# pingcap/tidb

Hardware: NVIDIA H100
Metric: hash-join probe rows/sec (higher is better)
Workload: dtype int64

## Files before the change

### tidb_b200/csrc/join.cu

```cuda
#include <memory>
#include <deque>
#include <algorithm>
#include <cmath>
#include <condition_variable>
#include "join_kernels.cuh"
#include "partition_kernels.cuh"
#include "chunk_io.cuh"

namespace tg {

static const int64_t kGeneralBatchRows = 16ll << 20;
static const int64_t kDirectPushRows = 128ll << 10;
static const int64_t kNextWindowRows = 1ll << 20;

struct Side {
  int ncols = 0;
  std::vector<int> types;
  std::vector<uint32_t> flags;
  std::vector<int> elem;
  std::vector<int> kelem;
  bool has_cells = false;
  std::vector<char> needed;
  int key_col = -1;
  std::vector<int> key_cols;
// ... 358 lines not shown
  return TG_OK;
}

static int kernel_view(JoinImpl* j, const Side& s, DevCols& v, int64_t rows) {
  if (!s.has_cells) return TG_OK;
  TG_TRY(ensure_iota(j, rows));
  for (int c = 0; c < s.ncols; c++)
    if (s.needed[c] && s.elem[c] == kCellBytes) { v.data[c] = j->iota.p; v.elem_len[c] = 8; }
  return TG_OK;
}

struct ProbeTuning { int ctas_per_sm; bool partition; int parts; int part_min_mb; int part_min_rows; int inplace; };
static ProbeTuning probe_tuning() {
  ProbeTuning t;
  t.ctas_per_sm = env_int("TG_PROBE_CTAS_PER_SM", 0);
  t.partition = env_int("TG_PROBE_PARTITION", 1) != 0;
  t.parts = env_int("TG_PROBE_PARTS", 0);
  t.part_min_mb = env_int("TG_PROBE_PART_MIN_MB", 64);
  t.part_min_rows = env_int("TG_PROBE_PART_MIN_ROWS", 1 << 22);
  t.inplace = env_int("TG_PROBE_INPLACE", -1);
  return t;
}

static size_t l2_slice_target(int device) {
  static size_t cache[64];
  if (device >= 0 && device < 64 && cache[device]) return cache[device];
  int l2 = 0;
  if (cudaDeviceGetAttribute(&l2, cudaDevAttrL2CacheSize, device) != cudaSuccess || l2 <= 0) { cudaGetLastError(); l2 = 50 << 20; }
  const size_t t = (size_t)l2 / 4;
  if (device >= 0 && device < 64) cache[device] = t;
  return t;
}
static int probe_slices(size_t table_bytes, int device, int parts_override) {
  if (parts_override > 0) return std::min(parts_override, TG_MAX_PARTS);
  const size_t target = l2_slice_target(device);
  return (int)std::min<size_t>((table_bytes + target - 1) / target, TG_MAX_PARTS);
}
static const double kMaxDenseLoad = 0.5;
static const double kInplaceMinMatch = 0.995;

static const double kPidxLoad = 0.7;
static const double kPidxKeysPerBucket = 4.0;
static const size_t kPidxMaxPilotBytes = 160 << 10;
static int enqueue_scan(JoinImpl* j, int64_t n, int64_t* nblocks_out);
static int build_slice_index(JoinImpl* j, const Slot* slots, unsigned long long nslots) {
  const ProbeTuning& tune = probe_tuning();
  const uint32_t P = (uint32_t)probe_slices((size_t)nslots * sizeof(Slot), j->device, tune.parts);
  if (P < 2) return TG_OK;
  DevBuf cnt;
  TG_TRY(cnt.ensure(j->device, (size_t)(TG_MAX_PARTS + 1) * 8));
  unsigned long long* pcnt = cnt.as<unsigned long long>();
  TG_CUDA(cudaMemsetAsync(pcnt, 0, (size_t)(TG_MAX_PARTS + 1) * 8, j->stream));
  k_pidx_part_count<<<grid_size(j->nsm, (int64_t)nslots, 256, 8), 256, 0, j->stream>>>(slots, nslots, P, pcnt);
  unsigned long long hc[TG_MAX_PARTS];
  TG_CUDA(cudaMemcpyAsync(hc, pcnt, P * 8, cudaMemcpyDeviceToHost, j->stream));
  TG_CUDA(cudaStreamSynchronize(j->stream));
  unsigned long long mx = 0;
  for (uint32_t p = 0; p < P; p++) mx = std::max(mx, hc[p]);
  SliceIndex ix{};
  ix.P = P;
  ix.S = (uint32_t)std::ceil((double)mx / kPidxLoad) + 1;
  ix.B = ((uint32_t)std::ceil((double)mx / kPidxKeysPerBucket) + 16) & ~15u;
  int optin = 0;
  cudaDeviceGetAttribute(&optin, cudaDevAttrMaxSharedMemoryPerBlockOptin, j->device);
  if (ix.B > kPidxMaxPilotBytes || ix.B > (uint32_t)optin) return TG_OK;
  const size_t nb = (size_t)P * ix.B, ns = (size_t)P * ix.S;
  TG_TRY(j->pidx_slots.ensure(j->device, ns * sizeof(Slot)));
  TG_TRY(j->pidx_pilot.ensure(j->device, nb));
  DevBuf owner, list;
  TG_TRY(owner.ensure(j->device, ns * 4));
  TG_TRY(list.ensure(j->device, (size_t)(mx * P + 1) * 4));
  TG_TRY(j->tmp_cnt.ensure(j->device, (nb + 1) * 4));
  Slot* islots = j->pidx_slots.as<Slot>();
  ix.slots = islots;
  ix.pilot = j->pidx_pilot.as<uint8_t>();
  TG_CUDA(cudaMemsetAsync(j->pidx_pilot.p, (int)kPilotNone, nb, j->stream));
  TG_CUDA(cudaMemsetAsync(owner.p, 0xFF, ns * 4, j->stream));
  TG_CUDA(cudaMemsetAsync(j->tmp_cnt.p, 0, (nb + 1) * 4, j->stream));
  k_table_init<<<grid_size(j->nsm, (int64_t)ns, 256, 8), 256, 0, j->stream>>>(islots, ns, ns);
  const unsigned g = (unsigned)grid_size(j->nsm, (int64_t)nslots, 256, 8);
  k_pidx_bucket_count<<<g, 256, 0, j->stream>>>(slots, nslots, ix, j->tmp_cnt.as<uint32_t>());
  int64_t nblocks = 0;
  TG_TRY(enqueue_scan(j, (int64_t)nb, &nblocks));
  const unsigned long long* off = j->tmp_off.as<unsigned long long>();
  k_pidx_lists<<<g, 256, 0, j->stream>>>(slots, nslots, ix, off, j->tmp_cnt.as<uint32_t>(), list.as<uint32_t>());
  const unsigned gb = (unsigned)grid_size(j->nsm, (int64_t)nb, 256, 8);
  for (uint32_t size = kPidxMaxBucket; size >= 1; size--)
    k_pidx_place<<<gb, 256, 0, j->stream>>>(slots, ix, off, list.as<uint32_t>(), size, owner.as<uint32_t>(), j->pidx_pilot.as<uint8_t>());
  unsigned long long* bad = pcnt + TG_MAX_PARTS;
  k_pidx_write<<<g, 256, 0, j->stream>>>(slots, nslots, ix, islots, 0, bad);
  k_pidx_write<<<g, 256, 0, j->stream>>>(slots, nslots, ix, islots, 1, bad);
  j->stats.kernel_launches += 8 + kPidxMaxBucket;
  unsigned long long hbad = 0;
  TG_CUDA(cudaMemcpyAsync(&hbad, bad, 8, cudaMemcpyDeviceToHost, j->stream));
  TG_CUDA(cudaStreamSynchronize(j->stream));
  if (hbad) { j->pidx_slots.release(); j->pidx_pilot.release(); return TG_OK; }
  j->pidx = ix;
  return TG_OK;
}


static int64_t inplace_seg_cap(const JoinImpl* j, int P, int64_t n_main, int64_t C0) {
  if (j->seg_parts != P || j->seg_rows <= 0) return C0;
  const double f = (double)j->seg_fill_max * (double)n_main / (double)j->seg_rows;
  const int64_t C = ((int64_t)(f + 8.0 * std::sqrt(f)) + 4096 + 127) / 128 * 128;
  return std::min(C, C0);
}

static int build_table(JoinImpl* j) {
  const Side& b = j->build;
  int64_t n = j->bcols.rows;
  j->stats.build_rows = n;
  DevCols bview = j->bcols.view(b);
  TG_TRY(kernel_view(j, b, bview, n));
  KeySpec ks = j->build_key;
  if (j->multi_key) {
    TG_TRY(composite_key(j, b, bview, n, j->bkey_syn, j->bkey_syn_nn));
    ks.data = j->bkey_syn.p; ks.nulls = j->bkey_syn_nn.as<uint8_t>();
  } else { ks.data = bview.data[b.key_col]; ks.nulls = bview.nulls[b.key_col]; }
  unsigned long long nslots = (unsigned long long)((double)(n > 0 ? n : 1) / j->load_factor) + 32;
  if (j->default_load_factor) {
    const unsigned long long fit = ((unsigned long long)TG_MAX_PARTS * (33ull << 20)) / sizeof(Slot);
// ... 307 lines not shown
};
template <int NPC, int NKD, int NMD>
struct LaunchSeg {
  static int run(JoinImpl* j, const int64_t* pkey, int64_t n, const FastOut& fo, unsigned long long* cur, const ProbeTuning& t, const SegSpec& seg) {
    static int resident = 0;
    if (!resident) {
      int nb = 0;
      if (cudaOccupancyMaxActiveBlocksPerMultiprocessor(&nb, k_probe_inner_u1_seg_lean<NPC, NKD, NMD>, 256, 0) != cudaSuccess || nb < 1) { cudaGetLastError(); nb = 3; }
      resident = nb;
    }
    int64_t ctas = (n / 128 + 7) / 8;
    int per_sm = t.ctas_per_sm > 0 ? t.ctas_per_sm : resident;
    int grid = (int)std::min<int64_t>(ctas, (int64_t)j->nsm * per_sm);
    k_probe_inner_u1_seg_lean<NPC, NKD, NMD><<<grid, 256, 0, j->stream>>>(pkey, n, j->tv, fo, cur, seg);
    return TG_OK;
  }
};
template <int NPC, int NKD, int NMD>
struct LaunchInplace {
  static int run(JoinImpl* j, int64_t n, const FastOut& fo, unsigned long long* cur, const ProbeTuning& t, const SegSpec& seg, uint32_t* tile_cnt) {
    if constexpr (NKD == 0) {
      return fail(TG_ERR_CUDA, "internal: the in-place segment probe needs an output fed by the join key");
    } else {
      static int resident = 0;
      if (!resident) {
        int nb = 0;
        if (cudaOccupancyMaxActiveBlocksPerMultiprocessor(&nb, k_probe_inner_u1_seg_inplace<NPC, NKD, NMD>, 256, 0) != cudaSuccess || nb < 1) { cudaGetLastError(); nb = 3; }
        resident = nb;
      }
      int64_t ctas = (n / 128 + 7) / 8;
      int per_sm = t.ctas_per_sm > 0 ? t.ctas_per_sm : resident;
      int grid = (int)std::min<int64_t>(ctas, (int64_t)j->nsm * per_sm);
      if (j->pidx.P == (uint32_t)(n / seg.cap)) {
        TG_CUDA(cudaFuncSetAttribute(k_probe_inner_u1_seg_inplace_pidx<NPC, NKD, NMD>, cudaFuncAttributeMaxDynamicSharedMemorySize,
                                     (int)kPidxMaxPilotBytes));
        k_probe_inner_u1_seg_inplace_pidx<NPC, NKD, NMD><<<j->nsm, kPidxThreads, j->pidx.B, j->stream>>>(n, j->tv, j->pidx, fo, cur, seg, tile_cnt);
        j->stats.paths |= TG_JOIN_PATH_PROBE_INDEX;
        return TG_OK;
      }
      k_probe_inner_u1_seg_inplace<NPC, NKD, NMD><<<grid, 256, 0, j->stream>>>(n, j->tv, fo, cur, seg, tile_cnt);
      return TG_OK;
    }
  }
};
static int launch_probe_warp(JoinImpl* j, const int64_t* pkey, int64_t n, const FastOut& fo, unsigned long long* cur, const ProbeTuning& t,
                             const SegSpec& seg = SegSpec{nullptr, 0, 0, 0, nullptr}) {
  j->stats.paths |= TG_JOIN_PATH_PROBE_DIRECT;
  return dispatch_shape<LaunchWarp>(fo, j, pkey, n, fo, cur, t, seg);
}
static int launch_probe_seg(JoinImpl* j, const int64_t* pkey, int64_t n, const FastOut& fo, unsigned long long* cur, const ProbeTuning& t, const SegSpec& seg) {
  j->stats.paths |= TG_JOIN_PATH_PROBE_SEG;
  return dispatch_shape<LaunchSeg>(fo, j, pkey, n, fo, cur, t, seg);
}
static bool aligned16(const void* p) { return (reinterpret_cast<uintptr_t>(p) & 15) == 0; }

static int probe_device(JoinImpl* j, const DevCols& pcells, int64_t n, ResultBatch& rb, bool sync_count, const SegSpec* in_seg = nullptr) {
  const Side& p = j->probe;
  DevCols pview = pcells;
  TG_TRY(kernel_view(j, p, pview, n));
  j->stats.probe_rows += n;
  KeySpec ks = j->probe_key;
  if (j->multi_key) {
    if (in_seg) return fail(TG_ERR_UNSUPPORTED, "segmented device chunks: joins on several key columns take the general path");
    TG_TRY(composite_key(j, p, pview, n, j->pkey_syn, j->pkey_syn_nn));
    ks.data = j->pkey_syn.p; ks.nulls = j->pkey_syn_nn.as<uint8_t>();
  } else { ks.data = pview.data[p.key_col]; ks.nulls = pview.nulls[p.key_col]; }
  TG_TRY(j->out_cursor.ensure(j->device, 64));
  OutCols oc{};
  fill_outspec_probe(j, oc);
// ... 2 lines not shown
  if (in_seg && !fast) return fail(TG_ERR_UNSUPPORTED, "segmented device chunks are only accepted by the fused fast path (unique build keys, <= 1 payload, no filters, an output shape the warp kernels cover)");
  if (fast) {
    const ProbeTuning& tune = probe_tuning();
    const int64_t* pkey = reinterpret_cast<const int64_t*>(ks.data);
    const size_t table_bytes = (size_t)j->tv.nslots * sizeof(Slot);
    bool src16 = aligned16(pkey);
    for (int c = 0; c < fo.n_pcols; c++) src16 = src16 && aligned16(fo.psrc[c]);
    const int64_t PTILE = 1024;
    const int64_t n_main = n / PTILE * PTILE;
    int P = 0;
    int64_t C = 0;
    if (n_main > 0 && tune.partition && src16 && n >= (int64_t)tune.part_min_rows && table_bytes > ((size_t)tune.part_min_mb << 20)) {
      P = probe_slices(table_bytes, j->device, tune.parts);
      C = ((int64_t)((double)n_main / P * 1.05) + 16384 + 127) / 128 * 128;
      if (!(P >= 2 && (int64_t)P * C / 128 < (1ll << 31))) P = 0;
    }
    const bool inplace = P && !in_seg && rb.rows == 0 && fo.n_key_dst >= 1 &&
                         (tune.inplace >= 0 ? tune.inplace != 0 : j->seg_match >= kInplaceMinMatch);
    if (inplace) C = inplace_seg_cap(j, P, n_main, C);
    TG_TRY(ensure_result(j, rb, inplace ? std::max<int64_t>(n, (int64_t)P * C) : rb.rows + n, rb.rows > 0, rb.rows));
    for (int c = 0; c < j->n_out; c++) { oc.data[c] = kernel_out(j, rb, c) + (size_t)rb.rows * 8; oc.valid[c] = nullptr; if (rb.bitmaps[c]->p) rb.bitmaps[c]->release(); }
    build_fast_out(j, oc, pview, fo);
    unsigned long long* cur = j->out_cursor.as<unsigned long long>();
    TG_CUDA(cudaMemsetAsync(cur, 0, 8, j->stream));
    if (n > 0) {
      if (P) {
        const int nc = 1 + fo.n_pcols;
        if (!inplace) {
          for (int c = 0; c < nc; c++) {
            if (!j->part_cols[c]) j->part_cols[c].reset(new DevBuf());
            TG_TRY(j->part_cols[c]->ensure(j->device, (size_t)P * C * 8 + 64));
          }
        }
        TG_TRY(j->part_scratch.ensure(j->device, (size_t)3 * TG_MAX_PARTS * 8 + 64));
        unsigned long long* cursors = j->part_scratch.as<unsigned long long>();
        long long* bases = reinterpret_cast<long long*>(cursors + TG_MAX_PARTS);
        unsigned long long* flag = cursors + 2 * TG_MAX_PARTS;
        PartDst d{};
        d.nparts = P; d.ncols = nc;
        d.src[0] = pkey;
        for (int c = 0; c < fo.n_pcols; c++) d.src[1 + c] = fo.psrc[c];
        for (int c = 0; c < nc; c++)
          for (int q = 0; q < P; q++) d.dst[q][c] = inplace ? (c == 0 ? (void*)fo.key_dst[0] : (void*)fo.pdst[c - 1]) : j->part_cols[c]->p;
        k_segment_bases<<<1, 32, 0, j->stream>>>(cursors, bases, flag, P, C);
        d.dst_base = bases; d.capacity = C; d.overflow = flag;
        if (in_seg) { d.in_cnt = in_seg->cnt; d.in_cap = in_seg->cap; d.in_tiles_per_seg = (uint32_t)(in_seg->cap / PTILE); }
        TG_TRY(launch_partition_scatter<true>(j->device, j->stream, reinterpret_cast<const long long*>(pkey), nullptr, n_main, d, cursors,
                                              &j->stats.kernel_launches, 0, &j->stats.paths));
        const SegSpec seg{cursors, (uint32_t)(C / 128), 0, C, flag};
        if (inplace) {
          const int64_t ntiles = (int64_t)P * C / 128;
          TG_TRY(j->tile_cnt.ensure(j->device, (size_t)ntiles * 4 + 16));
          TG_TRY(j->tmp_cnt.ensure(j->device, (size_t)(2 * ntiles + 1) * 4));
          j->stats.paths |= TG_JOIN_PATH_PROBE_SEG;
          TG_TRY(dispatch_shape<LaunchInplace>(fo, j, (int64_t)P * C, fo, cur, tune, seg, j->tile_cnt.as<uint32_t>()));
          k_inplace_holes<<<grid_size(j->nsm, ntiles, 256, 4), 256, 0, j->stream>>>(j->tile_cnt.as<uint32_t>(), ntiles, cur, flag, j->tmp_cnt.as<uint32_t>());
          int64_t nblocks = 0;
          TG_TRY(enqueue_scan(j, 2 * ntiles, &nblocks));
          k_inplace_fill<<<j->nsm * 8, 256, 0, j->stream>>>(j->tile_cnt.as<uint32_t>(), ntiles, j->tmp_off.as<unsigned long long>(), cur, flag, fo);
          j->stats.kernel_launches += 3;
        } else {
          FastOut pf = fo;
          for (int c = 0; c < fo.n_pcols; c++) pf.psrc[c] = j->part_cols[1 + c]->as<unsigned long long>();
          TG_TRY(launch_probe_seg(j, j->part_cols[0]->as<int64_t>(), (int64_t)P * C, pf, cur, tune, seg));
          j->stats.kernel_launches++;
        }
        if (in_seg) TG_TRY(launch_probe_warp(j, pkey, n_main, fo, cur, tune, SegSpec{in_seg->cnt, in_seg->tiles_per_seg, 1, in_seg->cap, flag, 0}));
        else TG_TRY(launch_probe_warp(j, pkey, n, fo, cur, tune, SegSpec{nullptr, 0, 1, 0, flag, n_main < n ? n_main : 0}));
        j->stats.kernel_launches += 2;
      } else {
        if (in_seg) TG_TRY(launch_probe_warp(j, pkey, n, fo, cur, tune, SegSpec{in_seg->cnt, in_seg->tiles_per_seg, 0, in_seg->cap, nullptr}));
        else TG_TRY(launch_probe_warp(j, pkey, n, fo, cur, tune));
        j->stats.kernel_launches++;
      }
    }
    TG_TRY(gather_cells(j, rb, &pcells, cur));
    if (sync_count) {
      unsigned long long got = 0, part[2 * TG_MAX_PARTS + 1];
      const bool learn = P && !in_seg;
      if (learn) TG_CUDA(cudaMemcpyAsync(part, j->part_scratch.p, sizeof(part), cudaMemcpyDeviceToHost, j->stream));
      TG_CUDA(cudaMemcpyAsync(&got, cur, 8, cudaMemcpyDeviceToHost, j->stream));
      TG_CUDA(cudaStreamSynchronize(j->stream));
      rb.rows += (int64_t)got;
      j->stats.output_rows += (int64_t)got;
      if (P && n > 0) j->seg_match = (double)got / (double)n;
      if (learn) {
        j->seg_parts = part[2 * TG_MAX_PARTS] ? 0 : P;
        j->seg_rows = n_main;
        j->seg_fill_max = (int64_t)*std::max_element(part, part + P);
      }
    }
    return TG_OK;
  }
  if (uq_path_ok(j, pview)) {
    TG_TRY(ensure_result(j, rb, rb.rows + n, rb.rows > 0, rb.rows));
    for (int c = 0; c < j->n_out; c++) { oc.data[c] = kernel_out(j, rb, c) + (size_t)rb.rows * 8; oc.valid[c] = nullptr; if (rb.bitmaps[c]->p) rb.bitmaps[c]->release(); }
    unsigned long long* cur = j->out_cursor.as<unsigned long long>();
    TG_CUDA(cudaMemsetAsync(cur, 0, 8, j->stream));
    if (n > 0) {
      int64_t tiles = (n + 256 * UQ_R - 1) / (256 * UQ_R);
      int grid = (int)std::min<int64_t>(tiles, (int64_t)j->nsm * 8);
      k_probe_inner_uq<<<grid, 256, 0, j->stream>>>(ks, pview, p.filter, n, j->tv, oc, cur);
      j->stats.kernel_launches++;
      j->stats.paths |= TG_JOIN_PATH_PROBE_UQ;
    }
    TG_TRY(gather_cells(j, rb, &pcells, cur));
    unsigned long long got = 0;
    TG_CUDA(cudaMemcpyAsync(&got, cur, 8, cudaMemcpyDeviceToHost, j->stream));
    TG_CUDA(cudaStreamSynchronize(j->stream));
    TG_CUDA(cudaGetLastError());
    rb.rows += (int64_t)got;
    j->stats.output_rows += (int64_t)got;
    return TG_OK;
  }
  std::vector<char> nullable;
  out_nullable(j, pview, nullable);
  if ((int)j->tmp_valid.size() != j->n_out) { j->tmp_valid.clear(); for (int i = 0; i < j->n_out; i++) j->tmp_valid.emplace_back(new DevBuf()); }
  int64_t out_start = rb.rows;
  for (int64_t lo = 0; lo < n || (lo == 0 && n == 0); lo += kGeneralBatchRows) {
    int64_t m = std::min<int64_t>(kGeneralBatchRows, n - lo);
// ... 375 lines not shown
```

### tidb_b200/csrc/join_kernels.cuh

```cuda
#pragma once
#include "common.cuh"
#include "tma.cuh"

namespace tg {

struct __align__(16) Slot { int64_t key; unsigned long long meta; };

static const uint32_t kInvalidSlot = 0xFFFFFFFFu;
static const unsigned long long kCntMask = (1ull << 28) - 1;

enum { TABLE_NONE = 0, TABLE_U1 = 1, TABLE_G = 2 };
enum { KEY_I64 = 0, KEY_F64 = 1, KEY_F32 = 2, KEY_TIME = 3 };
enum { SRC_PROBE_COL = 0, SRC_BUILD_KEY = 1, SRC_BUILD_META = 2, SRC_BUILD_WORD = 3, SRC_FLAG = 4 };

struct KeySpec {
  const void* data;
  const uint8_t* nulls;
  int32_t kind;
  int32_t reject_negative;
};

struct TableView {
  Slot* slots;
  unsigned long long nslots;
// ... 675 lines not shown
#pragma unroll
            for (int d = 1; d < NKD; d++) __stcs(reinterpret_cast<ulonglong2*>(out.key_dst[d] + o), kk);
#pragma unroll
            for (int d = 0; d < NMD; d++) __stcs(reinterpret_cast<ulonglong2*>(out.meta_dst[d] + o), make_ulonglong2(meta[2 * g], meta[2 * g + 1]));
          }
        } else {
          unsigned long long pv[R][NP];
          inplace_load_pv<NPC>(base, out, pv, lane);
          unsigned bal[R];
#pragma unroll
          for (int j = 0; j < R; j++) {
            bal[j] = __ballot_sync(0xffffffffu, (hit >> j) & 1u);
            m += __popc(bal[j]);
          }
          inplace_store<NPC, NKD, NMD>(base, k, meta, pv, bal, out, lane);
        }
      }
    } else if (limit > base) {
      m = inplace_tile_generic<NPC, NKD, NMD>(base, limit, t, out, lane);
    }
    if (lane == 0) tile_cnt[tile] = m;
    kept += m;
  }
  if (lane == 0 && kept) atomicAdd(out_cursor, kept);
}

static constexpr uint32_t kPilotNone = 255;
static constexpr int kPidxMaxBucket = 32;
static constexpr int kPidxThreads = 1024;

struct SliceIndex {
  const Slot* slots;
  const uint8_t* pilot;
  uint32_t P, S, B, pad;
};

__host__ __device__ __forceinline__ uint32_t pidx_slot(uint64_t h, uint32_t q, uint32_t S) {
  return slot32(hash64(h ^ ((uint64_t)(q + 1) * 0xC2B2AE3D27D4EB4Full)), S);
}
__host__ __device__ __forceinline__ uint32_t pidx_bucket(uint64_t h, uint32_t B) { return mulhi32((uint32_t)h, B); }

__global__ void __launch_bounds__(256) k_pidx_part_count(const Slot* __restrict__ slots, unsigned long long nslots, uint32_t P,
                                                         unsigned long long* __restrict__ pcnt) {
  __shared__ unsigned int c[64];
  for (int i = threadIdx.x; i < 64; i += blockDim.x) c[i] = 0;
  __syncthreads();
  for (unsigned long long i = blockIdx.x * (unsigned long long)blockDim.x + threadIdx.x; i < nslots; i += (unsigned long long)gridDim.x * blockDim.x) {
    const int64_t k = slots[i].key;
    if (k != kEmptyKey) atomicAdd(&c[slot32(hash64((uint64_t)k), P)], 1u);
  }
  __syncthreads();
  for (int i = threadIdx.x; i < (int)P; i += blockDim.x) if (c[i]) atomicAdd(&pcnt[i], (unsigned long long)c[i]);
}

__global__ void __launch_bounds__(256) k_pidx_bucket_count(const Slot* __restrict__ slots, unsigned long long nslots, SliceIndex ix,
                                                           uint32_t* __restrict__ bcnt) {
  for (unsigned long long i = blockIdx.x * (unsigned long long)blockDim.x + threadIdx.x; i < nslots; i += (unsigned long long)gridDim.x * blockDim.x) {
    const int64_t k = slots[i].key;
    if (k == kEmptyKey) continue;
    const uint64_t h = hash64((uint64_t)k);
    atomicAdd(&bcnt[(size_t)slot32(h, ix.P) * ix.B + pidx_bucket(h, ix.B)], 1u);
  }
}

__global__ void __launch_bounds__(256) k_pidx_lists(const Slot* __restrict__ slots, unsigned long long nslots, SliceIndex ix,
                                                    const unsigned long long* __restrict__ off, uint32_t* __restrict__ bcnt,
                                                    uint32_t* __restrict__ list) {
// ... 16 lines not shown
    uint64_t h[kPidxMaxBucket];
    for (uint32_t j = 0; j < size; j++) h[j] = hash64((uint64_t)slots[list[o + j]].key);
    uint32_t* const base = owner + (b / ix.B) * ix.S;
    for (uint32_t q = 0; q < kPilotNone; q++) {
      uint32_t won = 0;
      for (; won < size; won++)
        if (atomicCAS(base + pidx_slot(h[won], q, ix.S), 0xFFFFFFFFu, (uint32_t)b) != 0xFFFFFFFFu) break;
      if (won == size) { pilot[b] = (uint8_t)q; break; }
      for (uint32_t j = 0; j < won; j++) atomicExch(base + pidx_slot(h[j], q, ix.S), 0xFFFFFFFFu);
    }
  }
}

__global__ void __launch_bounds__(256) k_pidx_write(const Slot* __restrict__ slots, unsigned long long nslots, SliceIndex ix,
                                                    Slot* __restrict__ islots, int check, unsigned long long* __restrict__ bad) {
  for (unsigned long long i = blockIdx.x * (unsigned long long)blockDim.x + threadIdx.x; i < nslots; i += (unsigned long long)gridDim.x * blockDim.x) {
    const Slot s = slots[i];
    if (s.key == kEmptyKey) continue;
    const uint64_t h = hash64((uint64_t)s.key);
    const uint32_t p = slot32(h, ix.P);
    const uint32_t q = ix.pilot[(size_t)p * ix.B + pidx_bucket(h, ix.B)];
    if (q == kPilotNone) continue;
    Slot* d = islots + (size_t)p * ix.S + pidx_slot(h, q, ix.S);
    if (!check) *d = s;
    else if (d->key != s.key || d->meta != s.meta) atomicAdd(bad, 1ull);
  }
}

template <int NPC, int NKD, int NMD>
__global__ void __launch_bounds__(kPidxThreads, 1)
k_probe_inner_u1_seg_inplace_pidx(int64_t n, TableView t, SliceIndex ix, FastOut out, unsigned long long* __restrict__ out_cursor,
                                  SegSpec seg, uint32_t* __restrict__ tile_cnt) {
  static_assert(NKD >= 1, "the probe key is read from the first key destination");
  constexpr int R = 4, G = 2, NP = NPC > 0 ? NPC : 1;
  extern __shared__ __align__(16) uint8_t spil[];
  if (seg.gate && ((*seg.gate != 0ull) != (seg.gate_want != 0))) return;
  const int lane = threadIdx.x & 31;
  const int64_t warps_total = (int64_t)gridDim.x * (kPidxThreads / 32);
  const int64_t warp_id = (int64_t)blockIdx.x * (kPidxThreads / 32) + (threadIdx.x >> 5);
  const int64_t* __restrict__ pkey = reinterpret_cast<const int64_t*>(out.key_dst[0]);
  const int nseg = (int)(n / 128 / seg.tiles_per_seg);
  unsigned long long kept = 0;
  for (int p = 0; p < nseg; p++) {
    __syncthreads();
    const uint4* src = reinterpret_cast<const uint4*>(ix.pilot + (size_t)p * ix.B);
    for (uint32_t i = threadIdx.x; i < ix.B / 16; i += kPidxThreads) reinterpret_cast<uint4*>(spil)[i] = __ldcs(src + i);
    __syncthreads();
    const unsigned long long c = seg.cnt[p];
    const int64_t limit = (int64_t)p * seg.cap + (int64_t)(c < (unsigned long long)seg.cap ? c : (unsigned long long)seg.cap);
    const int64_t t0 = (int64_t)p * seg.tiles_per_seg, t1 = t0 + seg.tiles_per_seg;
    const Slot* __restrict__ islots = ix.slots + (size_t)p * ix.S;
    for (int64_t tile = t0 + warp_id; tile < t1; tile += warps_total) {
      const int64_t base = tile * 128;
      uint32_t m = 0;
      if (limit - base >= 128) {
        int64_t k[R];
#pragma unroll
        for (int g = 0; g < G; g++) {
          const ulonglong2 kk = __ldcs(reinterpret_cast<const ulonglong2*>(pkey + base + g * 64 + 2 * lane));
          k[2 * g] = (int64_t)kk.x; k[2 * g + 1] = (int64_t)kk.y;
        }
        uint32_t q[R];
        bool generic = false;
#pragma unroll
        for (int j = 0; j < R; j++) {
          q[j] = spil[pidx_bucket(hash64((uint64_t)k[j]), ix.B)];
          generic |= (k[j] == kEmptyKey) | (q[j] == kPilotNone);
        }
        if (__any_sync(0xffffffffu, generic)) {
          m = inplace_tile_generic<NPC, NKD, NMD>(base, limit, t, out, lane);
        } else {
          unsigned long long meta[R];
          unsigned hit = 0;
#pragma unroll
          for (int j = 0; j < R; j++) {
            const Slot v = load_slot(islots + pidx_slot(hash64((uint64_t)k[j]), q[j], ix.S));
            meta[j] = v.meta;
            if (v.key == k[j]) hit |= 1u << j;
          }
          if (__all_sync(0xffffffffu, hit == 0xFu)) {
            m = 128;
#pragma unroll
            for (int g = 0; g < G; g++) {
              const int64_t o = base + g * 64 + 2 * lane;
              const ulonglong2 kk = make_ulonglong2((unsigned long long)k[2 * g], (unsigned long long)k[2 * g + 1]);
#pragma unroll
              for (int d = 1; d < NKD; d++) __stcs(reinterpret_cast<ulonglong2*>(out.key_dst[d] + o), kk);
#pragma unroll
              for (int d = 0; d < NMD; d++) __stcs(reinterpret_cast<ulonglong2*>(out.meta_dst[d] + o), make_ulonglong2(meta[2 * g], meta[2 * g + 1]));
            }
          } else {
            unsigned long long pv[R][NP];
            inplace_load_pv<NPC>(base, out, pv, lane);
            unsigned bal[R];
#pragma unroll
            for (int j = 0; j < R; j++) {
              bal[j] = __ballot_sync(0xffffffffu, (hit >> j) & 1u);
              m += __popc(bal[j]);
            }
            inplace_store<NPC, NKD, NMD>(base, k, meta, pv, bal, out, lane);
          }
        }
      } else if (limit > base) {
        m = inplace_tile_generic<NPC, NKD, NMD>(base, limit, t, out, lane);
      }
      if (lane == 0) tile_cnt[tile] = m;
      kept += m;
    }
  }
  if (lane == 0 && kept) atomicAdd(out_cursor, kept);
}

__global__ void __launch_bounds__(256)
k_inplace_holes(const uint32_t* __restrict__ tile_cnt, int64_t ntiles, const unsigned long long* out_cursor,
                const unsigned long long* gate, uint32_t* __restrict__ cnt) {
  if (*gate) return;
  const int64_t R = (int64_t)*out_cursor;
  for (int64_t t = blockIdx.x * (int64_t)blockDim.x + threadIdx.x; t < ntiles; t += (int64_t)gridDim.x * blockDim.x) {
    const int64_t s = t * 128, e = s + tile_cnt[t];
    cnt[t] = e < R ? (uint32_t)((s + 128 < R ? s + 128 : R) - e) : 0u;
    cnt[ntiles + t] = e > R ? (uint32_t)(e - (s > R ? s : R)) : 0u;
  }
}

__device__ __forceinline__ int64_t last_le(const unsigned long long* __restrict__ off, int64_t lo, int64_t hi, unsigned long long k) {
  while (lo < hi) {
    const int64_t mid = (lo + hi + 1) >> 1;
    if (off[mid] <= k) lo = mid; else hi = mid - 1;
  }
  return lo;
}

__global__ void __launch_bounds__(256)
k_inplace_fill(const uint32_t* __restrict__ tile_cnt, int64_t ntiles, const unsigned long long* __restrict__ off,
               const unsigned long long* out_cursor, const unsigned long long* gate, FastOut out) {
  if (*gate) return;
  const int lane = threadIdx.x & 31;
  const int64_t warps_total = (int64_t)gridDim.x * (blockDim.x >> 5);
  const int64_t warp_id = (int64_t)blockIdx.x * (blockDim.x >> 5) + (threadIdx.x >> 5);
  const int64_t R = (int64_t)*out_cursor;
  const unsigned long long holes = off[ntiles];
// ... 330 lines not shown
```

### tidb_b200/csrc/partition_kernels.cuh

```cuda
#pragma once
#include "common.cuh"
#include "tma.cuh"
#include <algorithm>
#include <cstdlib>

namespace tg {

#define TG_MAX_PARTS 16
#define TG_PART_MAX_COLS 8
#define PT_BLOCK 256
#define PT_ITEMS 8
#define PT_TILE (PT_BLOCK * PT_ITEMS)

struct PartDst {
  int32_t nparts, ncols;
  const void* src[TG_PART_MAX_COLS];
  void* dst[TG_MAX_PARTS][TG_PART_MAX_COLS];
  const long long* dst_base;
  long long base_const;
  long long capacity;
  unsigned long long* overflow;
  const unsigned long long* in_cnt;
  long long in_cap;
  uint32_t in_tiles_per_seg;
  void* spill[TG_PART_MAX_COLS];
  long long spill_cap;
  unsigned long long* spill_cursor;
};

template <bool HIGH>
__device__ __forceinline__ uint32_t row_part(const long long* key, const uint8_t* nulls, int64_t i, uint32_t nparts) {
  uint64_t h = (nulls && !bit_not_null(nulls, i)) ? hash64((uint64_t)i)
                                                   : hash64((uint64_t)__ldcs(key + i));
  return HIGH ? mulhi32((uint32_t)(h >> 32), nparts) : part_of(h, nparts);
}

template <bool HIGH>
__global__ void __launch_bounds__(256)
k_partition_count(const long long* __restrict__ key, const uint8_t* __restrict__ nulls, int64_t n, uint32_t nparts,
                  unsigned long long* __restrict__ counts) {
  __shared__ unsigned long long s_cnt[TG_MAX_PARTS];
  if (threadIdx.x < TG_MAX_PARTS) s_cnt[threadIdx.x] = 0;
  __syncthreads();
  unsigned int local[TG_MAX_PARTS];
#pragma unroll
  for (int p = 0; p < TG_MAX_PARTS; p++) local[p] = 0;
  int64_t i = blockIdx.x * (int64_t)blockDim.x + threadIdx.x;
  int64_t stride = (int64_t)gridDim.x * blockDim.x;
  for (; i < n; i += stride) {
    uint32_t p = row_part<HIGH>(key, nulls, i, nparts);
#pragma unroll
    for (int q = 0; q < TG_MAX_PARTS; q++) local[q] += (p == (uint32_t)q);
  }
#pragma unroll
  for (int p = 0; p < TG_MAX_PARTS; p++) {
    unsigned int v = local[p];
    for (int o = 16; o; o >>= 1) v += __shfl_xor_sync(0xffffffffu, v, o);
    if ((threadIdx.x & 31) == 0 && v) atomicAdd(&s_cnt[p], (unsigned long long)v);
  }
  __syncthreads();
  if (threadIdx.x < nparts && s_cnt[threadIdx.x]) atomicAdd(&counts[threadIdx.x], s_cnt[threadIdx.x]);
}

static __global__ void k_partition_offsets(const unsigned long long* counts, uint32_t nparts, long long* part_offsets,
                                    unsigned long long* cursors) {
  if (threadIdx.x == 0 && blockIdx.x == 0) {
    long long run = 0;
    for (uint32_t p = 0; p < nparts; p++) { part_offsets[p] = run; cursors[p] = 0; run += (long long)counts[p]; }
    part_offsets[nparts] = run;
  }
}

static __global__ void k_segment_bases(unsigned long long* cursors, long long* bases, unsigned long long* flag, int nparts, long long cap) {
  if (threadIdx.x < TG_MAX_PARTS) { cursors[threadIdx.x] = 0; bases[threadIdx.x] = (long long)threadIdx.x * cap; }
  if (threadIdx.x == 0) *flag = 0;
  (void)nparts;
}

template <bool HIGH>
__global__ void __launch_bounds__(PT_BLOCK)
k_partition_scatter(const long long* __restrict__ key, const uint8_t* __restrict__ nulls, int64_t n, PartDst d,
                    unsigned long long* __restrict__ cursors) {
  __shared__ unsigned long long s_val[PT_TILE];
  __shared__ uint32_t s_cnt[TG_MAX_PARTS], s_off[TG_MAX_PARTS + 1], s_room[TG_MAX_PARTS];
  __shared__ unsigned long long s_gbase[TG_MAX_PARTS], s_spill[TG_MAX_PARTS];
  const int lane = threadIdx.x & 31;
  const uint32_t P = (uint32_t)d.nparts;
  const int64_t ntiles = (n + PT_TILE - 1) / PT_TILE;
  for (int64_t tile = blockIdx.x; tile < ntiles; tile += gridDim.x) {
    const int64_t base = tile * PT_TILE;
    if (threadIdx.x < TG_MAX_PARTS) s_cnt[threadIdx.x] = 0;
    __syncthreads();
    uint32_t part[PT_ITEMS], rank[PT_ITEMS];
#pragma unroll
    for (int j = 0; j < PT_ITEMS; j++) {
      int64_t i = base + (int64_t)j * PT_BLOCK + threadIdx.x;
      bool in = i < n;
      uint32_t p = in ? row_part<HIGH>(key, nulls, i, P) : 0xffffffffu;
      unsigned peers = __match_any_sync(0xffffffffu, p);
      uint32_t r = 0;
      if (in) {
        int leader = __ffs(peers) - 1;
        uint32_t wbase = 0;
        if (lane == leader) wbase = atomicAdd(&s_cnt[p], (uint32_t)__popc(peers));
        wbase = __shfl_sync(peers, wbase, leader);
        r = wbase + __popc(peers & ((1u << lane) - 1));
      }
      part[j] = p; rank[j] = r;
    }
    __syncthreads();
    if (threadIdx.x == 0) {
      uint32_t run = 0;
      for (uint32_t p = 0; p < P; p++) { s_off[p] = run; run += s_cnt[p]; }
      s_off[P] = run;
    }
    if (threadIdx.x < P) {
      uint32_t c = s_cnt[threadIdx.x];
      unsigned long long old = c ? atomicAdd(&cursors[threadIdx.x], (unsigned long long)c) : 0ull;
      s_gbase[threadIdx.x] = old + (unsigned long long)(d.dst_base ? d.dst_base[threadIdx.x] : d.base_const);
      unsigned long long room = d.capacity > 0 ? (old < (unsigned long long)d.capacity ? (unsigned long long)d.capacity - old : 0ull) : ~0ull;
      s_room[threadIdx.x] = room > c ? c : (uint32_t)room;
      unsigned long long sp = ~0ull;
      if (d.capacity > 0 && room < c) {
        if (d.spill_cursor) {
// ... 7 lines not shown
    __syncthreads();
    const uint32_t tile_rows = s_off[P];
    for (int c = 0; c < d.ncols; c++) {
      const unsigned long long* src = reinterpret_cast<const unsigned long long*>(d.src[c]);
#pragma unroll
      for (int j = 0; j < PT_ITEMS; j++) {
        int64_t i = base + (int64_t)j * PT_BLOCK + threadIdx.x;
        if (i < n) s_val[s_off[part[j]] + rank[j]] = __ldcs(src + i);
      }
      __syncthreads();
      for (uint32_t sidx = threadIdx.x; sidx < tile_rows; sidx += PT_BLOCK) {
        uint32_t p = 0;
        while (sidx >= s_off[p + 1]) p++;
        unsigned long long* dst = reinterpret_cast<unsigned long long*>(d.dst[p][c]);
        if (sidx - s_off[p] < s_room[p]) dst[s_gbase[p] + (sidx - s_off[p])] = s_val[sidx];
        else if (s_spill[p] != ~0ull) reinterpret_cast<unsigned long long*>(d.spill[c])[s_spill[p] + (sidx - s_off[p] - s_room[p])] = s_val[sidx];
      }
      __syncthreads();
    }
  }
}


__device__ __forceinline__ void bulk_s2g(void* dst_gmem, const void* src_smem, uint32_t bytes) {
  asm volatile("cp.async.bulk.global.shared::cta.bulk_group [%0], [%1], %2;" ::"l"(dst_gmem), "r"(smem_u32(src_smem)), "r"(bytes) : "memory");
}
__device__ __forceinline__ void bulk_commit() { asm volatile("cp.async.bulk.commit_group;" ::: "memory"); }
__device__ __forceinline__ void bulk_wait_read_all() { asm volatile("cp.async.bulk.wait_group.read 0;" ::: "memory"); }
__device__ __forceinline__ void fence_async_smem() { asm volatile("fence.proxy.async.shared::cta;" ::: "memory"); }

template <bool HIGH, int NC, int ITEMS>
__global__ void __launch_bounds__(PT_BLOCK)
k_partition_scatter_bulk(int64_t ntiles, PartDst d, unsigned long long* __restrict__ cursors) {
  constexpr int STAGES = 2, TILE = PT_BLOCK * ITEMS, SROWS = TILE + 2 * TG_MAX_PARTS;
  extern __shared__ __align__(128) unsigned char smem_raw[];
  unsigned long long* ring = reinterpret_cast<unsigned long long*>(smem_raw);
  unsigned long long* stage = ring + (size_t)STAGES * NC * TILE;
  uint64_t* full = reinterpret_cast<uint64_t*>(stage + (size_t)NC * SROWS);
  __shared__ uint32_t s_cnt[TG_MAX_PARTS], s_off[TG_MAX_PARTS], s_len[TG_MAX_PARTS];
  __shared__ unsigned long long s_gbase[TG_MAX_PARTS], s_spg[TG_MAX_PARTS];
  __shared__ uint32_t s_spn[TG_MAX_PARTS];
  const int tid = threadIdx.x, lane = tid & 31;
  const uint32_t P = (uint32_t)d.nparts;
  const unsigned long long pol = l2_policy_evict_first();
  if (tid == 0) {
    for (int s = 0; s < STAGES; s++) mbar_init(&full[s], 1);
    mbar_fence_init();
  }
  __syncthreads();
  auto issue = [&](int64_t it) {
    int64_t tile = (int64_t)blockIdx.x + it * gridDim.x;
    if (tile >= ntiles) return;
    int s = (int)(it % STAGES);
    mbar_arrive_expect_tx(&full[s], (uint32_t)(NC * TILE * 8));
#pragma unroll
    for (int c = 0; c < NC; c++)
      bulk_g2s(ring + ((size_t)s * NC + c) * TILE, reinterpret_cast<const unsigned long long*>(d.src[c]) + tile * TILE, TILE * 8, &full[s], pol);
  };
  if (tid == 0) for (int it = 0; it < STAGES; it++) issue(it);
  for (int64_t it = 0;; it++) {
    const int64_t tile = (int64_t)blockIdx.x + it * gridDim.x;
    if (tile >= ntiles) break;
    const int s = (int)(it % STAGES);
    if (tid < TG_MAX_PARTS) s_cnt[tid] = 0;
    mbar_wait(&full[s], (uint32_t)((it / STAGES) & 1));
    __syncthreads();
    const unsigned long long* in = ring + (size_t)s * NC * TILE;
    int valid = TILE;
    if (d.in_cnt) {
      const uint32_t sg = (uint32_t)tile / d.in_tiles_per_seg;
      const unsigned long long c = d.in_cnt[sg];
      const long long left = (long long)sg * d.in_cap + (long long)(c < (unsigned long long)d.in_cap ? c : (unsigned long long)d.in_cap) - tile * TILE;
      valid = left <= 0 ? 0 : (left < TILE ? (int)left : TILE);
    }
    uint32_t pr[ITEMS];
#pragma unroll
    for (int j = 0; j < ITEMS; j++) {
      if (j * PT_BLOCK + tid < valid) {
        uint64_t h = hash64(in[j * PT_BLOCK + tid]);
        uint32_t p = HIGH ? mulhi32((uint32_t)(h >> 32), P) : part_of(h, P);
        pr[j] = (p << 16) | atomicAdd(&s_cnt[p], 1u);
      } else pr[j] = 0xffffffffu;
    }
    __syncthreads();
    if (tid < 32) {
      uint32_t c = tid < (int)P ? s_cnt[tid] : 0, len = c, spn = 0;
      unsigned long long g = 0, spg = 0;
      if (tid < (int)P) {
        unsigned long long old = c ? atomicAdd(&cursors[tid], (unsigned long long)c) : 0ull;
        if (d.capacity > 0) {
          unsigned long long avail = old < (unsigned long long)d.capacity ? (unsigned long long)d.capacity - old : 0ull;
          if ((unsigned long long)c > avail) {
            len = (uint32_t)avail;
            if (d.spill_cursor) {
              spn = c - len;
              spg = atomicAdd(d.spill_cursor, (unsigned long long)spn);
              if (spg + spn > (unsigned long long)d.spill_cap) { spn = 0; *d.overflow = 1ull; }
// ... 90 lines not shown
  }
  __syncthreads();
  if (threadIdx.x < nparts && s_cnt[threadIdx.x]) atomicAdd(&counts[threadIdx.x], s_cnt[threadIdx.x]);
}


inline bool ptr_aligned16(const void* p) { return (reinterpret_cast<uintptr_t>(p) & 15) == 0; }

template <bool HIGH>
inline int launch_partition_count(int device, cudaStream_t st, const long long* key, const uint8_t* nulls, int64_t n, uint32_t nparts,
                                  unsigned long long* counts, int64_t* launches) {
  if (n <= 0) return TG_OK;
  int nsm = device_sm_count(device);
  if (!nulls && ptr_aligned16(key)) {
    int64_t need = ((n + 7) / 8 + 255) / 256;
    int grid = (int)std::min<int64_t>(std::max<int64_t>(need, 1), (int64_t)nsm * 8);
    k_partition_count4<HIGH><<<grid, 256, 0, st>>>(key, n, nparts, counts);
  } else {
    int64_t need = (n + 255) / 256;
    int grid = (int)std::min<int64_t>(std::max<int64_t>(need, 1), (int64_t)nsm * 8);
    k_partition_count<HIGH><<<grid, 256, 0, st>>>(key, nulls, n, nparts, counts);
  }
  if (launches) (*launches)++;
  return TG_OK;
}

template <bool HIGH, int NC>
inline int launch_scatter_nc(int device, cudaStream_t st, int64_t n, PartDst& d, unsigned long long* cursors, int64_t* launches, int ctas_per_sm,
                             int32_t* paths) {
  int nsm = device_sm_count(device);
  constexpr int ITEMS = 4, TILE = PT_BLOCK * ITEMS;
  int64_t ntiles = n / TILE;
  if (ntiles > 0) {
    size_t smem = (size_t)2 * NC * TILE * 8 + (size_t)NC * (TILE + 2 * TG_MAX_PARTS) * 8 + 2 * 8 + 16;
    TG_CUDA(cudaFuncSetAttribute(k_partition_scatter_bulk<HIGH, NC, ITEMS>, cudaFuncAttributeMaxDynamicSharedMemorySize, (int)smem));
    int per_sm = (int)std::max<size_t>(1, std::min<size_t>(4, (size_t)(220 * 1024) / (smem + 1024)));
    const int cap_env = env_int("TG_SCATTER_CTAS_PER_SM", 0);
    if (!HIGH && cap_env > 0 && per_sm > cap_env) per_sm = cap_env;
    if (ctas_per_sm > 0 && per_sm > ctas_per_sm) per_sm = ctas_per_sm;
    int grid = (int)std::min<int64_t>(ntiles, (int64_t)nsm * per_sm);
    k_partition_scatter_bulk<HIGH, NC, ITEMS><<<grid, PT_BLOCK, smem, st>>>(ntiles, d, cursors);
    if (launches) (*launches)++;
    if (paths) *paths |= TG_JOIN_PATH_SCATTER_BULK;
  }
  int64_t done = ntiles * TILE;
  if (done < n) {
    if (d.capacity > 0) return fail(TG_ERR_CUDA, "internal: capacity-bounded scatter needs a whole number of tiles");
    PartDst tail = d;
    for (int c = 0; c < NC; c++) tail.src[c] = reinterpret_cast<const unsigned long long*>(d.src[c]) + done;
    k_partition_scatter<HIGH><<<1, PT_BLOCK, 0, st>>>(reinterpret_cast<const long long*>(tail.src[0]), nullptr, n - done, tail, cursors);
    if (launches) (*launches)++;
  }
  return TG_OK;
}

template <bool HIGH>
inline int launch_partition_scatter(int device, cudaStream_t st, const long long* key, const uint8_t* nulls, int64_t n, PartDst& d,
                                    unsigned long long* cursors, int64_t* launches, int ctas_per_sm = 0, int32_t* paths = nullptr) {
  if (n <= 0) return TG_OK;
  bool tma_ok = !nulls && d.ncols <= 4 && d.src[0] == (const void*)key;
  for (int c = 0; c < d.ncols && tma_ok; c++) tma_ok = ptr_aligned16(d.src[c]);
  for (int p = 0; p < d.nparts && tma_ok; p++) for (int c = 0; c < d.ncols && tma_ok; c++) tma_ok = ptr_aligned16(d.dst[p][c]);
  if (tma_ok) {
    switch (d.ncols) {
      case 1: return launch_scatter_nc<HIGH, 1>(device, st, n, d, cursors, launches, ctas_per_sm, paths);
      case 2: return launch_scatter_nc<HIGH, 2>(device, st, n, d, cursors, launches, ctas_per_sm, paths);
      case 3: return launch_scatter_nc<HIGH, 3>(device, st, n, d, cursors, launches, ctas_per_sm, paths);
// ... 14 lines not shown
```

### tidb_b200/csrc/tma.cuh

```cuda
#pragma once
#include <cstdint>

namespace tg {

__device__ __forceinline__ uint32_t smem_u32(const void* p) { return (uint32_t)__cvta_generic_to_shared(p); }

__device__ __forceinline__ void mbar_init(uint64_t* bar, uint32_t count) {
  asm volatile("mbarrier.init.shared::cta.b64 [%0], %1;" ::"r"(smem_u32(bar)), "r"(count) : "memory");
}
__device__ __forceinline__ void mbar_fence_init() { asm volatile("fence.mbarrier_init.release.cluster;" ::: "memory"); }

__device__ __forceinline__ void mbar_arrive_expect_tx(uint64_t* bar, uint32_t bytes) {
  asm volatile("mbarrier.arrive.expect_tx.shared::cta.b64 _, [%0], %1;" ::"r"(smem_u32(bar)), "r"(bytes) : "memory");
}
__device__ __forceinline__ bool mbar_try_wait(uint64_t* bar, uint32_t parity) {
  uint32_t ok;
  asm volatile(
      "{\n"
      "  .reg .pred p;\n"
      "  mbarrier.try_wait.parity.shared::cta.b64 p, [%1], %2;\n"
      "  selp.u32 %0, 1, 0, p;\n"
      "}\n"
      : "=r"(ok)
      : "r"(smem_u32(bar)), "r"(parity)
      : "memory");
  return ok != 0;
}
__device__ __forceinline__ void mbar_wait(uint64_t* bar, uint32_t parity) {
  while (!mbar_try_wait(bar, parity)) {}
  __syncwarp();
}

__device__ __forceinline__ unsigned long long l2_policy_evict_first() {
  unsigned long long p;
  asm volatile("createpolicy.fractional.L2::evict_first.b64 %0, 1.0;" : "=l"(p));
  return p;
}
__device__ __forceinline__ unsigned long long l2_policy_evict_last() {
  unsigned long long p;
  asm volatile("createpolicy.fractional.L2::evict_last.b64 %0, 1.0;" : "=l"(p));
  return p;
}

__device__ __forceinline__ void bulk_g2s(void* dst_smem, const void* src_gmem, uint32_t bytes, uint64_t* bar,
                                         unsigned long long policy) {
  asm volatile(
      "cp.async.bulk.shared::cluster.global.mbarrier::complete_tx::bytes.L2::cache_hint [%0], [%1], %2, [%3], %4;"
      ::"r"(smem_u32(dst_smem)), "l"(src_gmem), "r"(bytes), "r"(smem_u32(bar)), "l"(policy)
      : "memory");
}

}
```

Baseline: 32.10 billion.

## Double-buffer pilot tables with TMA bulk loads in slice-index probe

Replaces the synchronous per-segment copy of the pilot table into shared memory with mbarrier-tracked cp.async.bulk loads into up to two buffers. The next segment's pilot is prefetched while warps probe the current one, and block-wide __syncthreads are removed in favour of per-warp completion counting. It also rotates each segment's starting warp so tail tiles spread across warps, and raises the override cap on slice count to 32, widening partition scratch arrays to match. The cost is extra shared memory per block, which can limit double buffering for large pilots, plus added barrier-protocol complexity.

```diff
diff --git a/tidb_b200/csrc/join.cu b/tidb_b200/csrc/join.cu
--- a/tidb_b200/csrc/join.cu
+++ b/tidb_b200/csrc/join.cu
@@ -414,7 +414,7 @@
   return t;
 }
 static int probe_slices(size_t table_bytes, int device, int parts_override) {
-  if (parts_override > 0) return std::min(parts_override, TG_MAX_PARTS);
+  if (parts_override > 0) return std::min(parts_override, TG_MAX_SLICES);
   const size_t target = l2_slice_target(device);
   return (int)std::min<size_t>((table_bytes + target - 1) / target, TG_MAX_PARTS);
 }
@@ -430,11 +430,11 @@
   const uint32_t P = (uint32_t)probe_slices((size_t)nslots * sizeof(Slot), j->device, tune.parts);
   if (P < 2) return TG_OK;
   DevBuf cnt;
-  TG_TRY(cnt.ensure(j->device, (size_t)(TG_MAX_PARTS + 1) * 8));
+  TG_TRY(cnt.ensure(j->device, (size_t)(TG_MAX_SLICES + 1) * 8));
   unsigned long long* pcnt = cnt.as<unsigned long long>();
-  TG_CUDA(cudaMemsetAsync(pcnt, 0, (size_t)(TG_MAX_PARTS + 1) * 8, j->stream));
+  TG_CUDA(cudaMemsetAsync(pcnt, 0, (size_t)(TG_MAX_SLICES + 1) * 8, j->stream));
   k_pidx_part_count<<<grid_size(j->nsm, (int64_t)nslots, 256, 8), 256, 0, j->stream>>>(slots, nslots, P, pcnt);
-  unsigned long long hc[TG_MAX_PARTS];
+  unsigned long long hc[TG_MAX_SLICES];
   TG_CUDA(cudaMemcpyAsync(hc, pcnt, P * 8, cudaMemcpyDeviceToHost, j->stream));
   TG_CUDA(cudaStreamSynchronize(j->stream));
   unsigned long long mx = 0;
@@ -445,7 +445,8 @@
   ix.B = ((uint32_t)std::ceil((double)mx / kPidxKeysPerBucket) + 16) & ~15u;
   int optin = 0;
   cudaDeviceGetAttribute(&optin, cudaDevAttrMaxSharedMemoryPerBlockOptin, j->device);
-  if (ix.B > kPidxMaxPilotBytes || ix.B > (uint32_t)optin) return TG_OK;
+  if (ix.B > kPidxMaxPilotBytes || ix.B + 16 > (uint32_t)optin) return TG_OK;
+  ix.nbuf = 2 * ix.B <= kPidxMaxPilotBytes && 2 * (ix.B + 8) <= (uint32_t)optin ? 2 : 1;
   const size_t nb = (size_t)P * ix.B, ns = (size_t)P * ix.S;
   TG_TRY(j->pidx_slots.ensure(j->device, ns * sizeof(Slot)));
   TG_TRY(j->pidx_pilot.ensure(j->device, nb));
@@ -469,7 +470,7 @@
   const unsigned gb = (unsigned)grid_size(j->nsm, (int64_t)nb, 256, 8);
   for (uint32_t size = kPidxMaxBucket; size >= 1; size--)
     k_pidx_place<<<gb, 256, 0, j->stream>>>(slots, ix, off, list.as<uint32_t>(), size, owner.as<uint32_t>(), j->pidx_pilot.as<uint8_t>());
-  unsigned long long* bad = pcnt + TG_MAX_PARTS;
+  unsigned long long* bad = pcnt + TG_MAX_SLICES;
   k_pidx_write<<<g, 256, 0, j->stream>>>(slots, nslots, ix, islots, 0, bad);
   k_pidx_write<<<g, 256, 0, j->stream>>>(slots, nslots, ix, islots, 1, bad);
   j->stats.kernel_launches += 8 + kPidxMaxBucket;
@@ -843,9 +844,9 @@
       int per_sm = t.ctas_per_sm > 0 ? t.ctas_per_sm : resident;
       int grid = (int)std::min<int64_t>(ctas, (int64_t)j->nsm * per_sm);
       if (j->pidx.P == (uint32_t)(n / seg.cap)) {
-        TG_CUDA(cudaFuncSetAttribute(k_probe_inner_u1_seg_inplace_pidx<NPC, NKD, NMD>, cudaFuncAttributeMaxDynamicSharedMemorySize,
-                                     (int)kPidxMaxPilotBytes));
-        k_probe_inner_u1_seg_inplace_pidx<NPC, NKD, NMD><<<j->nsm, kPidxThreads, j->pidx.B, j->stream>>>(n, j->tv, j->pidx, fo, cur, seg, tile_cnt);
+        const int smem = (int)(j->pidx.nbuf * (j->pidx.B + 8));
+        TG_CUDA(cudaFuncSetAttribute(k_probe_inner_u1_seg_inplace_pidx<NPC, NKD, NMD>, cudaFuncAttributeMaxDynamicSharedMemorySize, smem));
+        k_probe_inner_u1_seg_inplace_pidx<NPC, NKD, NMD><<<j->nsm, kPidxThreads, smem, j->stream>>>(n, j->tv, j->pidx, fo, cur, seg, tile_cnt);
         j->stats.paths |= TG_JOIN_PATH_PROBE_INDEX;
         return TG_OK;
       }
@@ -914,10 +915,10 @@
             TG_TRY(j->part_cols[c]->ensure(j->device, (size_t)P * C * 8 + 64));
           }
         }
-        TG_TRY(j->part_scratch.ensure(j->device, (size_t)3 * TG_MAX_PARTS * 8 + 64));
+        TG_TRY(j->part_scratch.ensure(j->device, (size_t)3 * TG_MAX_SLICES * 8 + 64));
         unsigned long long* cursors = j->part_scratch.as<unsigned long long>();
-        long long* bases = reinterpret_cast<long long*>(cursors + TG_MAX_PARTS);
-        unsigned long long* flag = cursors + 2 * TG_MAX_PARTS;
+        long long* bases = reinterpret_cast<long long*>(cursors + TG_MAX_SLICES);
+        unsigned long long* flag = cursors + 2 * TG_MAX_SLICES;
         PartDst d{};
         d.nparts = P; d.ncols = nc;
         d.src[0] = pkey;
@@ -958,7 +959,7 @@
     }
     TG_TRY(gather_cells(j, rb, &pcells, cur));
     if (sync_count) {
-      unsigned long long got = 0, part[2 * TG_MAX_PARTS + 1];
+      unsigned long long got = 0, part[2 * TG_MAX_SLICES + 1];
       const bool learn = P && !in_seg;
       if (learn) TG_CUDA(cudaMemcpyAsync(part, j->part_scratch.p, sizeof(part), cudaMemcpyDeviceToHost, j->stream));
       TG_CUDA(cudaMemcpyAsync(&got, cur, 8, cudaMemcpyDeviceToHost, j->stream));
@@ -967,7 +968,7 @@
       j->stats.output_rows += (int64_t)got;
       if (P && n > 0) j->seg_match = (double)got / (double)n;
       if (learn) {
-        j->seg_parts = part[2 * TG_MAX_PARTS] ? 0 : P;
+        j->seg_parts = part[2 * TG_MAX_SLICES] ? 0 : P;
         j->seg_rows = n_main;
         j->seg_fill_max = (int64_t)*std::max_element(part, part + P);
       }
diff --git a/tidb_b200/csrc/join_kernels.cuh b/tidb_b200/csrc/join_kernels.cuh
--- a/tidb_b200/csrc/join_kernels.cuh
+++ b/tidb_b200/csrc/join_kernels.cuh
@@ -731,7 +731,8 @@
 struct SliceIndex {
   const Slot* slots;
   const uint8_t* pilot;
-  uint32_t P, S, B, pad;
+  uint32_t P, S, B;
+  uint32_t nbuf;
 };
 
 __host__ __device__ __forceinline__ uint32_t pidx_slot(uint64_t h, uint32_t q, uint32_t S) {
@@ -814,25 +815,42 @@
 k_probe_inner_u1_seg_inplace_pidx(int64_t n, TableView t, SliceIndex ix, FastOut out, unsigned long long* __restrict__ out_cursor,
                                   SegSpec seg, uint32_t* __restrict__ tile_cnt) {
   static_assert(NKD >= 1, "the probe key is read from the first key destination");
-  constexpr int R = 4, G = 2, NP = NPC > 0 ? NPC : 1;
+  constexpr int R = 4, G = 2, NP = NPC > 0 ? NPC : 1, NW = kPidxThreads / 32;
   extern __shared__ __align__(16) uint8_t spil[];
+  __shared__ uint32_t s_done[2];
   if (seg.gate && ((*seg.gate != 0ull) != (seg.gate_want != 0))) return;
   const int lane = threadIdx.x & 31;
-  const int64_t warps_total = (int64_t)gridDim.x * (kPidxThreads / 32);
-  const int64_t warp_id = (int64_t)blockIdx.x * (kPidxThreads / 32) + (threadIdx.x >> 5);
+  const int64_t warps_total = (int64_t)gridDim.x * NW;
+  const int64_t warp_id = (int64_t)blockIdx.x * NW + (threadIdx.x >> 5);
   const int64_t* __restrict__ pkey = reinterpret_cast<const int64_t*>(out.key_dst[0]);
   const int nseg = (int)(n / 128 / seg.tiles_per_seg);
+  const int nbuf = (int)ix.nbuf;
+  uint64_t* full = reinterpret_cast<uint64_t*>(spil + (size_t)nbuf * ix.B);
+  auto load = [&](int p) {
+    const int b = p % nbuf;
+    mbar_arrive_expect_tx(&full[b], ix.B);
+    bulk_g2s(spil + (size_t)b * ix.B, ix.pilot + (size_t)p * ix.B, ix.B, &full[b], l2_policy_evict_normal());
+  };
+  if (threadIdx.x == 0) {
+    s_done[0] = s_done[1] = 0;
+    for (int b = 0; b < nbuf; b++) mbar_init(&full[b], 1);
+    mbar_fence_init();
+  }
+  __syncthreads();
+  if (threadIdx.x == 0)
+    for (int p = 0; p < nbuf && p < nseg; p++) load(p);
   unsigned long long kept = 0;
   for (int p = 0; p < nseg; p++) {
-    __syncthreads();
-    const uint4* src = reinterpret_cast<const uint4*>(ix.pilot + (size_t)p * ix.B);
-    for (uint32_t i = threadIdx.x; i < ix.B / 16; i += kPidxThreads) reinterpret_cast<uint4*>(spil)[i] = __ldcs(src + i);
-    __syncthreads();
+    const int b = p % nbuf;
+    const uint32_t use = (uint32_t)(p / nbuf);
+    mbar_wait(&full[b], use & 1u);
+    const uint8_t* __restrict__ pil = spil + (size_t)b * ix.B;
     const unsigned long long c = seg.cnt[p];
     const int64_t limit = (int64_t)p * seg.cap + (int64_t)(c < (unsigned long long)seg.cap ? c : (unsigned long long)seg.cap);
     const int64_t t0 = (int64_t)p * seg.tiles_per_seg, t1 = t0 + seg.tiles_per_seg;
+    const int64_t r = t0 % warps_total;
     const Slot* __restrict__ islots = ix.slots + (size_t)p * ix.S;
-    for (int64_t tile = t0 + warp_id; tile < t1; tile += warps_total) {
+    for (int64_t tile = t0 + (warp_id >= r ? warp_id - r : warp_id - r + warps_total); tile < t1; tile += warps_total) {
       const int64_t base = tile * 128;
       uint32_t m = 0;
       if (limit - base >= 128) {
@@ -846,7 +864,7 @@
         bool generic = false;
 #pragma unroll
         for (int j = 0; j < R; j++) {
-          q[j] = spil[pidx_bucket(hash64((uint64_t)k[j]), ix.B)];
+          q[j] = pil[pidx_bucket(hash64((uint64_t)k[j]), ix.B)];
           generic |= (k[j] == kEmptyKey) | (q[j] == kPilotNone);
         }
         if (__any_sync(0xffffffffu, generic)) {
@@ -889,6 +907,8 @@
       if (lane == 0) tile_cnt[tile] = m;
       kept += m;
     }
+    __syncwarp();
+    if (lane == 0 && atomicAdd(&s_done[b], 1u) == (use + 1) * NW - 1 && p + nbuf < nseg) load(p + nbuf);
   }
   if (lane == 0 && kept) atomicAdd(out_cursor, kept);
 }
diff --git a/tidb_b200/csrc/partition_kernels.cuh b/tidb_b200/csrc/partition_kernels.cuh
--- a/tidb_b200/csrc/partition_kernels.cuh
+++ b/tidb_b200/csrc/partition_kernels.cuh
@@ -7,6 +7,7 @@
 namespace tg {
 
 #define TG_MAX_PARTS 16
+#define TG_MAX_SLICES 32
 #define TG_PART_MAX_COLS 8
 #define PT_BLOCK 256
 #define PT_ITEMS 8
@@ -15,7 +16,7 @@
 struct PartDst {
   int32_t nparts, ncols;
   const void* src[TG_PART_MAX_COLS];
-  void* dst[TG_MAX_PARTS][TG_PART_MAX_COLS];
+  void* dst[TG_MAX_SLICES][TG_PART_MAX_COLS];
   const long long* dst_base;
   long long base_const;
   long long capacity;
@@ -72,7 +73,7 @@
 }
 
 static __global__ void k_segment_bases(unsigned long long* cursors, long long* bases, unsigned long long* flag, int nparts, long long cap) {
-  if (threadIdx.x < TG_MAX_PARTS) { cursors[threadIdx.x] = 0; bases[threadIdx.x] = (long long)threadIdx.x * cap; }
+  if (threadIdx.x < TG_MAX_SLICES) { cursors[threadIdx.x] = 0; bases[threadIdx.x] = (long long)threadIdx.x * cap; }
   if (threadIdx.x == 0) *flag = 0;
   (void)nparts;
 }
@@ -82,14 +83,14 @@
 k_partition_scatter(const long long* __restrict__ key, const uint8_t* __restrict__ nulls, int64_t n, PartDst d,
                     unsigned long long* __restrict__ cursors) {
   __shared__ unsigned long long s_val[PT_TILE];
-  __shared__ uint32_t s_cnt[TG_MAX_PARTS], s_off[TG_MAX_PARTS + 1], s_room[TG_MAX_PARTS];
-  __shared__ unsigned long long s_gbase[TG_MAX_PARTS], s_spill[TG_MAX_PARTS];
+  __shared__ uint32_t s_cnt[TG_MAX_SLICES], s_off[TG_MAX_SLICES + 1], s_room[TG_MAX_SLICES];
+  __shared__ unsigned long long s_gbase[TG_MAX_SLICES], s_spill[TG_MAX_SLICES];
   const int lane = threadIdx.x & 31;
   const uint32_t P = (uint32_t)d.nparts;
   const int64_t ntiles = (n + PT_TILE - 1) / PT_TILE;
   for (int64_t tile = blockIdx.x; tile < ntiles; tile += gridDim.x) {
     const int64_t base = tile * PT_TILE;
-    if (threadIdx.x < TG_MAX_PARTS) s_cnt[threadIdx.x] = 0;
+    if (threadIdx.x < TG_MAX_SLICES) s_cnt[threadIdx.x] = 0;
     __syncthreads();
     uint32_t part[PT_ITEMS], rank[PT_ITEMS];
 #pragma unroll
@@ -163,14 +164,14 @@
 template <bool HIGH, int NC, int ITEMS>
 __global__ void __launch_bounds__(PT_BLOCK)
 k_partition_scatter_bulk(int64_t ntiles, PartDst d, unsigned long long* __restrict__ cursors) {
-  constexpr int STAGES = 2, TILE = PT_BLOCK * ITEMS, SROWS = TILE + 2 * TG_MAX_PARTS;
+  constexpr int STAGES = 2, TILE = PT_BLOCK * ITEMS, SROWS = TILE + 2 * TG_MAX_SLICES;
   extern __shared__ __align__(128) unsigned char smem_raw[];
   unsigned long long* ring = reinterpret_cast<unsigned long long*>(smem_raw);
   unsigned long long* stage = ring + (size_t)STAGES * NC * TILE;
   uint64_t* full = reinterpret_cast<uint64_t*>(stage + (size_t)NC * SROWS);
-  __shared__ uint32_t s_cnt[TG_MAX_PARTS], s_off[TG_MAX_PARTS], s_len[TG_MAX_PARTS];
-  __shared__ unsigned long long s_gbase[TG_MAX_PARTS], s_spg[TG_MAX_PARTS];
-  __shared__ uint32_t s_spn[TG_MAX_PARTS];
+  __shared__ uint32_t s_cnt[TG_MAX_SLICES], s_off[TG_MAX_SLICES], s_len[TG_MAX_SLICES];
+  __shared__ unsigned long long s_gbase[TG_MAX_SLICES], s_spg[TG_MAX_SLICES];
+  __shared__ uint32_t s_spn[TG_MAX_SLICES];
   const int tid = threadIdx.x, lane = tid & 31;
   const uint32_t P = (uint32_t)d.nparts;
   const unsigned long long pol = l2_policy_evict_first();
@@ -193,7 +194,7 @@
     const int64_t tile = (int64_t)blockIdx.x + it * gridDim.x;
     if (tile >= ntiles) break;
     const int s = (int)(it % STAGES);
-    if (tid < TG_MAX_PARTS) s_cnt[tid] = 0;
+    if (tid < TG_MAX_SLICES) s_cnt[tid] = 0;
     mbar_wait(&full[s], (uint32_t)((it / STAGES) & 1));
     __syncthreads();
     const unsigned long long* in = ring + (size_t)s * NC * TILE;
@@ -350,7 +351,7 @@
   constexpr int ITEMS = 4, TILE = PT_BLOCK * ITEMS;
   int64_t ntiles = n / TILE;
   if (ntiles > 0) {
-    size_t smem = (size_t)2 * NC * TILE * 8 + (size_t)NC * (TILE + 2 * TG_MAX_PARTS) * 8 + 2 * 8 + 16;
+    size_t smem = (size_t)2 * NC * TILE * 8 + (size_t)NC * (TILE + 2 * TG_MAX_SLICES) * 8 + 2 * 8 + 16;
     TG_CUDA(cudaFuncSetAttribute(k_partition_scatter_bulk<HIGH, NC, ITEMS>, cudaFuncAttributeMaxDynamicSharedMemorySize, (int)smem));
     int per_sm = (int)std::max<size_t>(1, std::min<size_t>(4, (size_t)(220 * 1024) / (smem + 1024)));
     const int cap_env = env_int("TG_SCATTER_CTAS_PER_SM", 0);
diff --git a/tidb_b200/csrc/tma.cuh b/tidb_b200/csrc/tma.cuh
--- a/tidb_b200/csrc/tma.cuh
+++ b/tidb_b200/csrc/tma.cuh
@@ -36,6 +36,11 @@
   asm volatile("createpolicy.fractional.L2::evict_first.b64 %0, 1.0;" : "=l"(p));
   return p;
 }
+__device__ __forceinline__ unsigned long long l2_policy_evict_normal() {
+  unsigned long long p;
+  asm volatile("createpolicy.fractional.L2::evict_normal.b64 %0, 1.0;" : "=l"(p));
+  return p;
+}
 __device__ __forceinline__ unsigned long long l2_policy_evict_last() {
   unsigned long long p;
   asm volatile("createpolicy.fractional.L2::evict_last.b64 %0, 1.0;" : "=l"(p));
```

After: 34.34 billion (median of 6 runs). +7.0%, better.
